# HaokunChen245/FedDAT

Hardware: AMD Instinct MI355X
Metric: VQA samples/sec, ViLT-B/32 dual-adapter local step (higher is better)
Workload: dtype fp16; 1 GPU; configs[1] with fp16 operands (BASELINE.json's configs[1] string says bf16: same operand width and MFMA rate; the bf16 step is in other_operand_format with --full): ViLT-B/32 FedDAT, 1 client per MI355X, fp16 MFMA operands (dynamic loss scale, GradScaler semantics on the device, initial 2^14), fp32 accumulate / masters, batch=32/client, 384x384 synthetic + 40-token questions, MKD on; batch_per_client=32, seq_len=185, clients=1, hip_graph=True, ranks=1, hetero_steps=False

## Files before the change

feddat_amd/csrc/common.hip.h:

```cpp
#pragma once
#include <hip/hip_runtime.h>
#include <stdint.h>

#include "../../include/feddat_hip.h"

typedef __bf16 tbf16;
typedef __bf16 tbf16x8 __attribute__((ext_vector_type(8)));
#ifdef FEDDAT_OPERANDS_F16
typedef _Float16 bf16;
#define FD_OPERAND_FORMAT FEDDAT_OPERANDS_FP16
#define FD_MFMA_16X16X32_ASM "v_mfma_f32_16x16x32_f16"
#else
typedef __bf16 bf16;
#define FD_OPERAND_FORMAT FEDDAT_OPERANDS_BF16
#define FD_MFMA_16X16X32_ASM "v_mfma_f32_16x16x32_bf16"
#endif
typedef bf16 bf16x2 __attribute__((ext_vector_type(2)));
typedef bf16 bf16x4 __attribute__((ext_vector_type(4)));
typedef bf16 bf16x8 __attribute__((ext_vector_type(8)));
typedef short s16x4 __attribute__((ext_vector_type(4)));
typedef float f32x4 __attribute__((ext_vector_type(4)));
typedef float f32x2 __attribute__((ext_vector_type(2)));

#define FD_WAVE 64

#if defined(__HIP_DEVICE_COMPILE__) && !defined(__gfx950__)
#error "libfeddat_hip.so is written for gfx950 (MI355X) only: build with --offload-arch=gfx950"
#endif

#define FD_CHECK_ARG(cond)                 \
    do {                                   \
        if (!(cond)) return FEDDAT_EINVAL; \
    } while (0)

#define FD_LAUNCH_RET()                                        \
    do {                                                       \
        hipError_t e__ = hipGetLastError();                    \
        return e__ == hipSuccess ? FEDDAT_OK : FEDDAT_ELAUNCH; \
    } while (0)

int fd_device_cus(int* n_cu);
int fd_set_max_lds(const void* kernel, int bytes);
#ifdef FEDDAT_ABLATE
#define FD_ABL(x) (x)
#else
#define FD_ABL(x) 0
#endif
constexpr unsigned FD_DEBUG_SELECT_BITS = 1u | 2u | 32u | 64u | 128u | 256u | (1u << 23) | (1u << 27) | (0xfu << 28);
int fd_debug_flags();
int fd_prepare_all_kernels();
int fd_prepare_gemm_kernels();
int fd_prepare_attn_kernels();

#define LDS_PTR(p) ((__attribute__((address_space(3))) void*)(p))
#define GLB_PTR(p) ((const __attribute__((address_space(1))) void*)(p))

__device__ __forceinline__ float wave_sum(float v) {
#pragma unroll
    for (int o = 32; o > 0; o >>= 1) v += __shfl_xor(v, o, 64);
    return v;
}
__device__ __forceinline__ float wave_max(float v) {
#pragma unroll
    for (int o = 32; o > 0; o >>= 1) v = fmaxf(v, __shfl_xor(v, o, 64));
    return v;
}
__device__ __forceinline__ bool fd_nonfinite(float x) { return !(fabsf(x) <= __FLT_MAX__); }

__device__ __forceinline__ uint32_t fd_fmix32(uint32_t x) {
    x ^= x >> 16; x *= 0x85EBCA6Bu; x ^= x >> 13; x *= 0xC2B2AE35u; x ^= x >> 16;
    return x;
}
struct FdDrop {
    uint32_t key0, key1s, thr;
    float scale;
};
__device__ __forceinline__ FdDrop fd_drop_make(float p, uint32_t key0, uint32_t key1, const int* step) {
    FdDrop d;
    d.key0 = key0;
    d.key1s = key1 + (step ? (uint32_t)*step : 0u) * 0x632BE5ABu;
    d.thr = (uint32_t)((double)p * 4294967296.0);
    d.scale = 1.0f / (1.0f - p);
    return d;
}
__device__ __forceinline__ bool fd_drop_keep(const FdDrop& d, uint32_t idx) {
    return fd_fmix32(fd_fmix32(idx * 0x9E3779B1u + d.key0) + d.key1s) >= d.thr;
}

__device__ __forceinline__ void erf_exp_f(float u, float& erf_x, float& exp_mx2) {
    const float x = u * 0.70710678118654752f;
    const float ax = fabsf(x);
    const float t = __frcp_rn(1.0f + 0.3275911f * ax);
    exp_mx2 = __expf(-x * x);
    const float poly = t * (0.254829592f + t * (-0.284496736f + t * (1.421413741f + t * (-1.453152027f + t * 1.061405429f))));
    const float e = 1.0f - poly * exp_mx2;
    erf_x = copysignf(e, x);
}
__device__ __forceinline__ float gelu_f(float u) {
    float er, ex;
    erf_exp_f(u, er, ex);
    return 0.5f * u * (1.0f + er);
}
__device__ __forceinline__ float gelu_grad_f(float u) {
    float er, ex;
    erf_exp_f(u, er, ex);
    return 0.5f * (1.0f + er) + u * 0.39894228040143268f * ex;
}

typedef float f32x2 __attribute__((ext_vector_type(2)));
__device__ __forceinline__ f32x2 odd_poly9_pk(f32x2 t, const float (&c)[9]) {
    const f32x2 t2 = t * t;
    f32x2 p = f32x2{c[8], c[8]};
#pragma unroll
    for (int k = 7; k >= 0; --k) p = p * t2 + f32x2{c[k], c[k]};
    return p * t;
}
__device__ __forceinline__ f32x2 clamp_unit_pk(f32x2 u) {
    f32x2 t = u * f32x2{1.0f / 4.5f, 1.0f / 4.5f};
    t[0] = __builtin_amdgcn_fmed3f(t[0], -1.0f, 1.0f);
    t[1] = __builtin_amdgcn_fmed3f(t[1], -1.0f, 1.0f);
    return t;
}
__device__ __forceinline__ f32x2 gelu_pk(f32x2 u) {
    constexpr float C[9] = {3.589798371e+00f, -1.207231863e+01f, 3.590728051e+01f, -8.046883329e+01f, 1.320808609e+02f,
                            -1.519935397e+02f, 1.145676310e+02f, -5.029529085e+01f, 9.684438904e+00f};
    const f32x2 e = odd_poly9_pk(clamp_unit_pk(u), C);
    const f32x2 h = u * f32x2{0.5f, 0.5f};
    return h * e + h;
}
__device__ __forceinline__ f32x2 gelu_grad_pk(f32x2 u) {
    constexpr float C[9] = {3.586068066e+00f, -2.393606056e+01f, 1.043871964e+02f, -2.983035769e+02f, 5.731157980e+02f,
// ... 106 lines not shown
```

feddat_amd/csrc/gemm_bf16.hip:

```cpp
#include <stdlib.h>

#include <type_traits>

#include "common.hip.h"

namespace {

constexpr int BM = 128, BN = 128, BK = 64;
typedef unsigned int u32x4 __attribute__((ext_vector_type(4)));
constexpr int TILE_BYTES = BM * BK * 2;

struct GemmArgs {
    const bf16* A;
    const bf16* B;
    const float* bias;
    const float* resid;
    const bf16* aux;
    float* out_f32;
    bf16* out_bf16;
    bf16* out2_bf16;
    int M, N, K;
    int lda, ldb, ldr, ldaux, ldo32, ldo16, ldo2;
    int epi;
    int nostore;
// ... 227 lines not shown
#pragma unroll
                    for (int j = 0; j < 2; ++j) fb[j] = read_frag(tb, wn * 32 + j * 16 + frow, ks * 4 + fg);
#pragma unroll
                    for (int i = 0; i < 2; ++i)
#pragma unroll
                        for (int j = 0; j < 2; ++j) acc[i][j] = mfma16x32(fb[j], fa[i], acc[i][j]);
                }
            }
            __syncthreads();
        }
    }
    tile_epilogue_dispatch<2, 2>(g, acc, m0 + wm * 32, n0 + wn * 32, g.M, lane);
}


constexpr int V2_BN = 192;
constexpr int V2_TILE_B = V2_BN * BK * 2;
constexpr int V2_EPI_WAVE = 5120;
constexpr int V2_EPI_LD = 208;
template <int WM> struct V2Cfg {
    static constexpr int BM = 64 * WM;
    static constexpr int TILE_A = BM * BK * 2;
    static constexpr int STAGE = TILE_A + V2_TILE_B;
    static constexpr int EPI_OFF = 2 * STAGE;
    static constexpr int LDS = EPI_OFF + 8 * V2_EPI_WAVE;
    static constexpr int NP = WM + 3;
};


struct GemmArgsV2 {
    GemmArgs g;
    int bm;
    int tiles_m;
    int nx, tm_per, tn_per;
    int dbg;
};

__device__ __forceinline__ void v2_tile_coords(const GemmArgsV2& a, int tile_id, int total, int& m0, int& n0,
                                               int& m_last) {
    const int tiles_n = a.g.N / V2_BN;
    int tm, tn;
    if (a.nx == 1) {
        const int q = total >> 3, r8 = total & 7, xcd = tile_id & 7;
        const int wg = (xcd < r8 ? xcd * (q + 1) : r8 * (q + 1) + (xcd - r8) * q) + (tile_id >> 3);
        tm = wg / tiles_n;
        tn = wg - tm * tiles_n;
    } else {
        const int xcd = tile_id & 7, li = tile_id >> 3;
        const int xm = xcd / a.nx, xn = xcd - xm * a.nx;
        const int lm = li / a.tn_per;
        tm = xm * a.tm_per + lm;
        tn = xn * a.tn_per + (li - lm * a.tn_per);
    }
    m0 = tm * a.bm;
    n0 = tn * V2_BN;
    m_last = min(m0 + a.bm, a.g.M) - 1;
}

template <int WM>
__device__ __forceinline__ void v2_piece_ptrs(const GemmArgs& g, int m0, int m_last, int n0, int wave, int lane,
                                              const bf16* (&pa)[WM], const bf16* (&pb)[3]) {
#pragma unroll
    for (int i = 0; i < WM; ++i) {
        const int r = (wave * WM + i) * 8 + (lane >> 3);
        pa[i] = g.A + (size_t)min(m0 + r, m_last) * g.lda + (lane & 7) * 8;
    }
#pragma unroll
    for (int i = 0; i < 3; ++i) {
        const int r = (wave * 3 + i) * 8 + (lane >> 3);
        pb[i] = g.B + (size_t)min(n0 + r, g.N - 1) * g.ldb + (lane & 7) * 8;
    }
}

constexpr int V2_EPI_LD16 = 208;
constexpr int V2_EPI_LD8 = 112;
#ifdef FD_EPI_NT
#define FD_STREAM_STORE(ptr, val) __builtin_nontemporal_store((val), (ptr))
#define FD_STREAM_LOAD(ptr) __builtin_nontemporal_load(ptr)
#else
#define FD_STREAM_STORE(ptr, val) (*(ptr) = (val))
#define FD_STREAM_LOAD(ptr) (*(ptr))
#endif
__device__ uint4 fd_epi_sink[64];
template <int EPI, int WM, bool SINK = false>
__device__ __forceinline__ void v2_epilogue_bf16(const GemmArgs& g, f32x4 (&acc)[WM][6], char* stg, int mbase, int nbase,
                                                 int m_end, int lane) {
    asm volatile("" : "+v"(lane));
    const int frow = lane & 15, fg = lane >> 4;
    constexpr bool G8OUT_ = EPI == FEDDAT_EPI_GELU_G8 || EPI == FEDDAT_EPI_MUL_G8 || EPI == FEDDAT_EPI_GELU_G8_F8 ||
                            EPI == FEDDAT_EPI_MUL_G8_F8;
    constexpr int COLC_OFF = 16 * V2_EPI_LD16;
    static_assert(COLC_OFF + 2 * 384 <= V2_EPI_WAVE, "column constants fit behind the staged slab");
    f32x4 bias4[G8OUT_ ? 1 : 6];
    if (G8OUT_) {
        if (lane < 24) {
            *reinterpret_cast<f32x4*>(stg + COLC_OFF + lane * 16) =
                g.bias ? *reinterpret_cast<const f32x4*>(g.bias + nbase + lane * 4) : f32x4{0.f, 0.f, 0.f, 0.f};
            if (g.sw) *reinterpret_cast<f32x4*>(stg + COLC_OFF + 384 + lane * 16) = *reinterpret_cast<const f32x4*>(g.sw + nbase + lane * 4);
        }
    } else {
#pragma unroll
        for (int j = 0; j < 6; ++j)
            bias4[j] = g.bias ? *reinterpret_cast<const f32x4*>(g.bias + nbase + j * 16 + fg * 4) : f32x4{0.f, 0.f, 0.f, 0.f};
    }
    int srow[3], sc8[3];
#pragma unroll
    for (int p = 0; p < 3; ++p) {
        const int idx = p * 64 + lane;
        srow[p] = idx / 12;
        sc8[p] = idx - srow[p] * 12;
    }
    constexpr bool G8OUT = EPI == FEDDAT_EPI_GELU_G8 || EPI == FEDDAT_EPI_GELU_G8_F8;
    constexpr bool G8IN = EPI == FEDDAT_EPI_MUL_G8 || EPI == FEDDAT_EPI_MUL_G8_F8;
    constexpr bool F8OUT = EPI == FEDDAT_EPI_GELU_G8_F8 || EPI == FEDDAT_EPI_MUL_G8_F8;
    int r8[2], c8[2];
#pragma unroll
    for (int p = 0; p < 2; ++p) {
        const int idx = p * 64 + lane;
        r8[p] = idx / 6;
        c8[p] = idx - r8[p] * 6;
    }
    char* wr8 = stg + frow * V2_EPI_LD8 + fg * 4;
    u32x4 ux8[G8IN ? WM : 1][2];
    auto aux8_load = [&](int i) {
#pragma unroll
        for (int p = 0; p < 2; ++p) {
            const unsigned mc = (unsigned)min(mbase + i * 16 + r8[p], m_end - 1);
            const unsigned off = mc * (unsigned)g.ldaux + (unsigned)(nbase + c8[p] * 16);
            ux8[i][p] = FD_STREAM_LOAD(reinterpret_cast<const u32x4*>(reinterpret_cast<const char*>(g.aux) + off));
        }
    };
    if (G8IN) {
#pragma unroll
        for (int i = 0; i < WM; ++i) aux8_load(i);
    }
    bf16x8 ux[G8IN ? 1 : WM][3];
    auto aux_load = [&](int i) {
#pragma unroll
        for (int p = 0; p < 3; ++p) {
            const unsigned mc = (unsigned)min(mbase + i * 16 + srow[p], m_end - 1);
            const unsigned off = (mc * (unsigned)g.ldaux + (unsigned)(nbase + sc8[p] * 8)) * 2u;
            ux[i][p] = *reinterpret_cast<const bf16x8*>(reinterpret_cast<const char*>(g.aux) + off);
        }
    };
    constexpr int AUX_AHEAD = WM < 4 ? WM : 4;
    if (EPI == FEDDAT_EPI_MUL_DGELU) {
#pragma unroll
        for (int i = 0; i < AUX_AHEAD; ++i) aux_load(i);
    }
    char* wr = stg + frow * V2_EPI_LD16 + fg * 8;
    auto put = [&](bf16* dst, int ld, int i, const f32x4 (&val)[6]) {
#pragma unroll
        for (int j = 0; j < 6; ++j) *reinterpret_cast<bf16x4*>(wr + j * 32) = cvt4(val[j]);
        bf16x8 v[3];
#pragma unroll
        for (int p = 0; p < 3; ++p) v[p] = *reinterpret_cast<const bf16x8*>(stg + srow[p] * V2_EPI_LD16 + sc8[p] * 16);
#pragma unroll
        for (int p = 0; p < 3; ++p) {
            const int m = mbase + i * 16 + srow[p];
            if (SINK) {
                bf16* o = m < m_end ? dst + (size_t)m * ld + nbase + sc8[p] * 8 : reinterpret_cast<bf16*>(fd_epi_sink) + lane * 8;
                *reinterpret_cast<bf16x8*>(o) = v[p];
            } else if (m < m_end && !FD_ABL(g.nostore & 1)) {
                FD_STREAM_STORE(reinterpret_cast<bf16x8*>(dst + (size_t)m * ld + nbase + sc8[p] * 8), v[p]);
            }
        }
    };
    auto slab8_out = [&](uint8_t* o8, int ld, int i) {
        u32x4 cv[2];
#pragma unroll
        for (int p = 0; p < 2; ++p) cv[p] = *reinterpret_cast<const u32x4*>(stg + r8[p] * V2_EPI_LD8 + c8[p] * 16);
#pragma unroll
        for (int p = 0; p < 2; ++p) {
            const int m = mbase + i * 16 + r8[p];
            if (m < m_end && (p == 0 || lane < 32) && !FD_ABL(g.nostore & 1))
                FD_STREAM_STORE(reinterpret_cast<u32x4*>(o8 + (size_t)m * ld + nbase + c8[p] * 16), cv[p]);
        }
    };
    f32x4 sw4[G8OUT_ ? 1 : 6];
    if (g.sw && !G8OUT_) {
#pragma unroll
        for (int j = 0; j < 6; ++j) sw4[j] = *reinterpret_cast<const f32x4*>(g.sw + nbase + j * 16 + fg * 4);
    }
    auto colc = [&](int which, int j) { return *reinterpret_cast<const f32x4*>(stg + COLC_OFF + which * 384 + j * 64 + fg * 16); };
#pragma unroll
    for (int i = 0; i < WM; ++i) {
        f32x4 val[6];
        if (g.sw) {
            const float sa = g.sa ? g.sa[min(mbase + i * 16 + frow, m_end - 1)] : 1.0f;
#pragma unroll
            for (int j = 0; j < 6; ++j) {
                if (EPI == FEDDAT_EPI_MUL_G8_F8)
                    val[j] = acc[i][j] * (colc(1, j) * f32x4{1.0f / FEDDAT_F8_GRAD_HEADROOM, 1.0f / FEDDAT_F8_GRAD_HEADROOM,
                                                              1.0f / FEDDAT_F8_GRAD_HEADROOM, 1.0f / FEDDAT_F8_GRAD_HEADROOM});
                else
                    val[j] = acc[i][j] * ((G8OUT_ ? colc(1, j) : sw4[j]) * f32x4{sa, sa, sa, sa}) + (G8OUT_ ? colc(0, j) : bias4[j]);
            }
        } else {
#pragma unroll
            for (int j = 0; j < 6; ++j) val[j] = acc[i][j] + (G8OUT_ ? colc(0, j) : bias4[j]);
        }
        if (EPI == FEDDAT_EPI_MUL_DGELU) {
#pragma unroll
            for (int p = 0; p < 3; ++p) *reinterpret_cast<bf16x8*>(stg + srow[p] * V2_EPI_LD16 + sc8[p] * 16) = ux[i][p];
#pragma unroll
            for (int j = 0; j < 6; ++j) {
                const bf16x4 u = *reinterpret_cast<const bf16x4*>(wr + j * 32);
                if (!FD_ABL(g.nostore & 2)) val[j] = val[j] * gelu_grad4_pk(f32x4{(float)u[0], (float)u[1], (float)u[2], (float)u[3]});
                else val[j] = val[j] * f32x4{(float)u[0], (float)u[1], (float)u[2], (float)u[3]};
            }
            if (i + AUX_AHEAD < WM) aux_load(i + AUX_AHEAD);
        }
        if (EPI == FEDDAT_EPI_GELU) {
            if (g.out2_bf16) put(g.out2_bf16, g.ldo2, i, val);
#pragma unroll
            for (int j = 0; j < 6; ++j)
                if (!FD_ABL(g.nostore & 2)) val[j] = gelu4_pk(val[j]);
        }
        if (G8IN) {
#pragma unroll
            for (int p = 0; p < 2; ++p) *reinterpret_cast<u32x4*>(stg + r8[p] * V2_EPI_LD8 + c8[p] * 16) = ux8[i][p];
#pragma unroll
            for (int j = 0; j < 6; ++j) val[j] = val[j] * fd_g8_decode4(*reinterpret_cast<const unsigned*>(wr8 + j * 16));
        }
        if (G8OUT) {
#pragma unroll
            for (int j = 0; j < 6; ++j) {
                f32x4 fj, gj;
                gelu_and_grad4_pk(val[j], fj, gj);
                *reinterpret_cast<unsigned*>(wr8 + j * 16) = fd_g8_encode4(FD_ABL(g.nostore & 2) ? val[j] : gj);
                val[j] = fj;
            }
            slab8_out(reinterpret_cast<uint8_t*>(g.out2_bf16), g.ldo2, i);
        }
        if (F8OUT) {
            constexpr float S = EPI == FEDDAT_EPI_GELU_G8_F8 ? 1.0f / FEDDAT_F8_ACT_SCALE : 1.0f;
#pragma unroll
            for (int j = 0; j < 6; ++j) {
                f32x4 x = val[j] * f32x4{S, S, S, S};
#pragma unroll
                for (int e = 0; e < 4; ++e) x[e] = __builtin_amdgcn_fmed3f(x[e], -448.0f, 448.0f);
                int pk = __builtin_amdgcn_cvt_pk_fp8_f32(x[0], x[1], 0, false);
                pk = __builtin_amdgcn_cvt_pk_fp8_f32(x[2], x[3], pk, true);
                *reinterpret_cast<int*>(wr8 + j * 16) = pk;
            }
            slab8_out(reinterpret_cast<uint8_t*>(g.out_bf16), g.ldo16, i);
        } else {
            put(g.out_bf16, g.ldo16, i, val);
        }
    }
}

template <int EPI, int WM, bool DEQ = false>
__device__ __forceinline__ void v2_epilogue(const GemmArgs& g, f32x4 (&acc)[WM][6], char* stg, int mbase, int nbase,
                                            int m_end, int lane) {
    asm volatile("" : "+v"(lane));
    const int frow = lane & 15, fg = lane >> 4;
    f32x4 bias4[6];
#pragma unroll
    for (int j = 0; j < 6; ++j)
        bias4[j] = g.bias ? *reinterpret_cast<const f32x4*>(g.bias + nbase + j * 16 + fg * 4) : f32x4{0.f, 0.f, 0.f, 0.f};
    f32x4 sw4[DEQ ? 6 : 1];
    if (DEQ) {
#pragma unroll
        for (int j = 0; j < 6; ++j) sw4[j] = *reinterpret_cast<const f32x4*>(g.sw + nbase + j * 16 + fg * 4);
    }
    int srow[3], sc4[3];
// ... 94 lines not shown
#endif
    const GemmArgs& g = a.g;
    const int tid = threadIdx.x;
    const int lane = tid & 63;
    const int wave = __builtin_amdgcn_readfirstlane(tid >> 6);
    const int grp = wave >> 2;
    const int wm = wave >> 1, wn = wave & 1;
    const int total = a.tiles_m * (g.N / V2_BN);
    const int grid = gridDim.x, bid = blockIdx.x;
    const int my_tiles = (total - bid + grid - 1) / grid;
    const int nk = g.K / BK;
    const int total_it = my_tiles * nk;

    f32x4 acc[WM][6];
#pragma unroll
    for (int i = 0; i < WM; ++i)
#pragma unroll
        for (int j = 0; j < 6; ++j) acc[i][j] = f32x4{0.f, 0.f, 0.f, 0.f};

    int m0, n0, m_last;
    v2_tile_coords(a, bid, total, m0, n0, m_last);
    V2State<WM> L;
    v2_piece_ptrs<WM>(g, m0, m_last, n0, wave, lane, L.pa, L.pb);
    auto sc_ptr = [&](int tm0, int tml) {
        const int r = wave * (8 * WM) + min(lane, 8 * WM - 1);
        return g.amx + (size_t)min(tm0 + r, tml) * g.ld_mx;
    };
    L.psc = MXA ? sc_ptr(m0, m_last) : nullptr;
    L.l_tile = 0;
    L.l_kt = 0;
    int issued = 0;
    const int lds_lane = (lane >> 3) * 128 + ((((lane & 7) ^ (lane >> 3)) & 7) << 4);

    u32x4 rs[NP];
    int written = 0;
    auto gload_piece = [&](int p) {
        const int koff = L.l_kt * BK;
        rs[p] = *reinterpret_cast<const u32x4*>((p < WM ? L.pa[p < WM ? p : 0] : L.pb[p < WM ? 0 : p - WM]) + koff);
    };
    auto stream_advance = [&]() {
        if (issued + 1 < total_it) {
            if (++L.l_kt == nk) {
                L.l_kt = 0;
                ++L.l_tile;
                int lm0, ln0, lml;
                v2_tile_coords(a, bid + L.l_tile * grid, total, lm0, ln0, lml);
                v2_piece_ptrs<WM>(g, lm0, lml, ln0, wave, lane, L.pa, L.pb);
                if (MXA) L.psc = sc_ptr(lm0, lml);
            }
        }
        ++issued;
    };
    auto lwrite_piece = [&](int p, int stage) {
        char* sb = smem + stage * Cfg::STAGE + lds_lane +
                   (p < WM ? (wave * WM + p) * 1024 : Cfg::TILE_A + (wave * 3 + p - WM) * 1024);
        *reinterpret_cast<u32x4*>(sb) = rs[p];
    };
    unsigned rsc = 0;
    auto gload_sc = [&]() {
        if (MXA) rsc = *reinterpret_cast<const unsigned*>(L.psc + L.l_kt * 4);
    };
    auto lwrite_sc = [&](int stage) {
        if (MXA && lane < 8 * WM) *reinterpret_cast<unsigned*>(smem + SC_OFF + stage * (256 * WM) + (wave * (8 * WM) + lane) * 4) = rsc;
    };
    auto gload = [&]() {
#pragma unroll
        for (int p = 0; p < NP; ++p) gload_piece(p);
        gload_sc();
        stream_advance();
    };
    auto lwrite = [&](int stage) {
#pragma unroll
        for (int p = 0; p < NP; ++p) lwrite_piece(p, stage);
        lwrite_sc(stage);
        ++written;
    };

    const int frow = lane & 15, fg = lane >> 4;
    const int frag_off[2] = {frow * 128 + (((0 + fg) ^ (frow & 7)) << 4), frow * 128 + (((4 + fg) ^ (frow & 7)) << 4)};
    char* stg = smem + Cfg::EPI_OFF + wave * V2_EPI_WAVE;
    int kt = 0, c_tile = 0, st = 0;
    bool pend = false;
    int pm0 = 0, pn0 = 0, pml = 0;
    auto run_epilogue = [&](int em0, int en0, int eml) {
        const int mb = em0 + wm * (16 * WM), nb = en0 + wn * 96, me = eml + 1;
        if (!FD_ABL(a.dbg & 8)) {
            if (EPI == FEDDAT_EPI_BF16 || EPI == FEDDAT_EPI_GELU || EPI == FEDDAT_EPI_MUL_DGELU || EPI == FEDDAT_EPI_GELU_G8 ||
                EPI == FEDDAT_EPI_MUL_G8 || EPI == FEDDAT_EPI_GELU_G8_F8 || EPI == FEDDAT_EPI_MUL_G8_F8)
                v2_epilogue_bf16<EPI, WM>(g, acc, stg, mb, nb, me, lane);
            else
                v2_epilogue<EPI, WM, FP8>(g, acc, stg, mb, nb, me, lane);
        }
#pragma unroll
        for (int i = 0; i < WM; ++i)
#pragma unroll
            for (int j = 0; j < 6; ++j) acc[i][j] = f32x4{0.f, 0.f, 0.f, 0.f};
    };

    gload();
    lwrite(0);
    gload();
    if (grp == 1) {
        lwrite(1);
        gload();
    }
    asm volatile("s_waitcnt lgkmcnt(0)" ::: "memory");
    __builtin_amdgcn_sched_barrier(0);
    __builtin_amdgcn_s_barrier();
    if (grp == 1) __builtin_amdgcn_s_barrier();
    __builtin_amdgcn_sched_barrier(0);

    for (int it = 0; it < total_it; ++it) {
        bf16x8 fa[2][WM], fb[2][6];
        int asc[MXA ? WM : 1];
        auto read_frags = [&]() {
            if (MXA) {
#pragma unroll
                for (int i = 0; i < WM; ++i)
                    asc[i] = *reinterpret_cast<const uint8_t*>(smem + SC_OFF + st * (256 * WM) + (wm * (16 * WM) + i * 16 + frow) * 4 + fg);
            }
            const int a_base = st * Cfg::STAGE + wm * (16 * WM * 128);
            const int b_base = st * Cfg::STAGE + Cfg::TILE_A + wn * (96 * 128);
#pragma unroll
            for (int ks = 0; ks < 2; ++ks) {
                const char* pb_ = smem + (frag_off[ks] + b_base);
                const char* pa_ = smem + (frag_off[ks] + a_base);
#pragma unroll
                for (int j = 0; j < 6; ++j) fb[ks][j] = *reinterpret_cast<const bf16x8*>(pb_ + j * 2048);
#pragma unroll
                for (int i = 0; i < WM; ++i) fa[ks][i] = *reinterpret_cast<const bf16x8*>(pa_ + i * 2048);
                __builtin_amdgcn_sched_barrier(0);
            }
        };
        const bool boundary = pend;
        if (boundary && grp == 0) {
            __builtin_amdgcn_sched_barrier(0);
            __builtin_amdgcn_s_barrier();
            __builtin_amdgcn_sched_barrier(0);
        }
        if (boundary) {
            run_epilogue(pm0, pn0, pml);
            pend = false;
            if (grp == 1) {
                __builtin_amdgcn_sched_barrier(0);
                __builtin_amdgcn_s_barrier();
                __builtin_amdgcn_sched_barrier(0);
            }
        }
        read_frags();
        asm volatile("s_waitcnt lgkmcnt(0)" ::: "memory");
        __builtin_amdgcn_sched_barrier(0);
        __builtin_amdgcn_s_barrier();
        __builtin_amdgcn_sched_barrier(0);
        const int wstage = written & 1;
        __builtin_amdgcn_s_setprio(1);
        if constexpr (FP8 && !FP8_K32) {
#pragma unroll
            for (int i = 0; i < WM; ++i) {
#pragma unroll
                for (int j = 0; j < 6; ++j)
                    acc[i][j] = MXA ? mfma16x128_fp8_mx_sb(fb[0][j], fb[1][j], fa[0][i], fa[1][i], acc[i][j], asc[MXA ? i : 0])
                                    : mfma16x128_fp8_mx(fb[0][j], fb[1][j], fa[0][i], fa[1][i], acc[i][j]);
                __builtin_amdgcn_sched_barrier(0);
#pragma unroll
                for (int p = 2 * i; p < 2 * i + 2; ++p)
                    if (p < NP) {
                        lwrite_piece(p, wstage);
                        gload_piece(p);
                    }
                if (MXA && i == WM - 1) {
                    lwrite_sc(wstage);
                    gload_sc();
                }
                __builtin_amdgcn_sched_barrier(0);
            }
        } else {
#pragma unroll
        for (int ks = 0; ks < 2; ++ks)
#pragma unroll
            for (int i = 0; i < WM; ++i) {
#pragma unroll
                for (int j = 0; j < 6; ++j)
                    acc[i][j] = FP8 ? mfma16x64_fp8(fb[ks][j], fa[ks][i], acc[i][j]) : mfma16x32(fb[ks][j], fa[ks][i], acc[i][j]);
                __builtin_amdgcn_sched_barrier(0);
                if (ks * WM + i < NP) {
                    lwrite_piece(ks * WM + i, wstage);
                    gload_piece(ks * WM + i);
                }
                __builtin_amdgcn_sched_barrier(0);
            }
        }
        __builtin_amdgcn_s_setprio(0);
        ++written;
        stream_advance();
        asm volatile("s_waitcnt lgkmcnt(0)" ::: "memory");
        st ^= 1;
        if (++kt == nk) {
            kt = 0;
            pend = true; pm0 = m0; pn0 = n0; pml = m_last;
            if (++c_tile < my_tiles) v2_tile_coords(a, bid + c_tile * grid, total, m0, n0, m_last);
        }
        __builtin_amdgcn_sched_barrier(0);
        __builtin_amdgcn_s_barrier();
        __builtin_amdgcn_sched_barrier(0);
    }
    if (grp == 0) __builtin_amdgcn_s_barrier();
    __builtin_amdgcn_sched_barrier(0);
    if (pend) run_epilogue(pm0, pn0, pml);
}





__device__ __forceinline__ void mfma_agpr(f32x4& c, const bf16x8& a, const bf16x8& b) {
    asm volatile(FD_MFMA_16X16X32_ASM " %0, %1, %2, %0" : "+a"(c) : "v"(a), "v"(b));
}
__device__ __forceinline__ void mfma_agpr_first(f32x4& c, const bf16x8& a, const bf16x8& b) {
    asm volatile(FD_MFMA_16X16X32_ASM " %0, %1, %2, 0" : "=a"(c) : "v"(a), "v"(b));
}

__device__ __forceinline__ void mfma_vgpr(f32x4& c, const bf16x8& a, const bf16x8& b) {
    asm volatile(FD_MFMA_16X16X32_ASM " %0, %1, %2, %0" : "+v"(c) : "v"(a), "v"(b));
}
__device__ __forceinline__ void mfma_vgpr_first(f32x4& c, const bf16x8& a, const bf16x8& b) {
    asm volatile(FD_MFMA_16X16X32_ASM " %0, %1, %2, 0" : "=v"(c) : "v"(a), "v"(b));
}

template <int RT> struct V3Cfg {
    static constexpr int BM = 32 * RT;
    static constexpr int TILE_A = BM * BK * 2;
    static constexpr int STAGE = TILE_A + V2_TILE_B;
    static constexpr int EPI_OFF = 2 * STAGE;
    static constexpr int LDS = EPI_OFF + 4 * V2_EPI_WAVE;
    static constexpr int NP = RT + 6;
};

template <int EPI, int RT, int FAKE = 0, bool DUAL = false>
__global__ __launch_bounds__(256, DUAL ? 2 : 1) void gemm_nt_v3_kernel(GemmArgsV2 a) {
    using Cfg = V3Cfg<RT>;
    static_assert(!DUAL || (RT == 4 && 4 * V2_EPI_WAVE <= Cfg::STAGE), "the dual form: 128-row tiles, staging inside one stage");
    constexpr int NP = Cfg::NP, NM = 6 * RT;
    constexpr int LH0 = (NM - 2 * NP) < NP ? (NM - 2 * NP) : NP;
    static_assert(LH0 >= 0 && NP - LH0 <= 12, "writes fit half 0, deferred reloads fit ahead of half 1's fragment reads");
    extern __shared__ __attribute__((aligned(16))) char smem[];
#ifdef FEDDAT_ABLATE
    if (const int q = (a.dbg >> 24) & 7) {
        const long t0 = wall_clock64(), d = (long)((blockIdx.x >> 3) & 3) * q * 200;
        while (wall_clock64() - t0 < d) __builtin_amdgcn_s_sleep(8);
    }
#endif
    const GemmArgs& g = a.g;
    const int tid = threadIdx.x;
    const int lane = tid & 63;
    const int wave = __builtin_amdgcn_readfirstlane(tid >> 6);
    const int wm = wave >> 1, wn = wave & 1;
    const int total = a.tiles_m * (g.N / V2_BN);
    const int grid = gridDim.x, bid = blockIdx.x;
    const int my_tiles = (total - bid + grid - 1) / grid;
    const int nk = g.K / BK;
    const int total_it = my_tiles * nk;

    f32x4 acc[RT][6];
    int m0, n0, m_last;
    v2_tile_coords(a, bid, total, m0, n0, m_last);
    unsigned pp[NP];
    auto piece_ptrs = [&](int tm0, int tml, int tn0) {
#pragma unroll
        for (int i = 0; i < RT; ++i) {
            const int r = (wave * RT + i) * 8 + (lane >> 3);
            pp[i] = ((unsigned)min(tm0 + r, tml) * (unsigned)g.lda + (lane & 7) * 8) * 2u;
        }
#pragma unroll
        for (int i = 0; i < 6; ++i) {
            const int r = (wave * 6 + i) * 8 + (lane >> 3);
            pp[RT + i] = ((unsigned)min(tn0 + r, g.N - 1) * (unsigned)g.ldb + (lane & 7) * 8) * 2u;
        }
    };
    piece_ptrs(m0, m_last, n0);
    int l_tile = 0, l_kt = 0, issued = 0;
    const int lds_lane = (lane >> 3) * 128 + ((((lane & 7) ^ (lane >> 3)) & 7) << 4);
    u32x4 rs[NP];
    auto gload_piece = [&](int p) {
        const char* base = reinterpret_cast<const char*>(p < RT ? g.A : g.B) + (size_t)l_kt * (BK * 2);
        rs[p] = *reinterpret_cast<const u32x4*>(base + pp[p]);
    };
    auto stream_advance = [&]() {
        if (issued + 1 < total_it) {
            if (++l_kt == nk) {
// ... 513 lines not shown
                                  const float* b_scale, int M, int N, int K, int epi, const float* bias, const void* aux,
                                  int ldaux, void* out_bf16, int ldo16, void* out2_bf16, int ldo2, hipStream_t stream) {
    FD_CHECK_ARG(A8 && B8 && a_scale && b_scale && out_bf16 && M >= 1024 && N > 0 && N % V2_BN == 0 && K > 0 && K % 128 == 0);
    const bool g8in = epi == FEDDAT_EPI_MUL_G8 || epi == FEDDAT_EPI_MUL_G8_F8;
    const bool g8out = epi == FEDDAT_EPI_GELU_G8 || epi == FEDDAT_EPI_GELU_G8_F8;
    const bool f8out = epi == FEDDAT_EPI_GELU_G8_F8 || epi == FEDDAT_EPI_MUL_G8_F8;
    FD_CHECK_ARG(epi == FEDDAT_EPI_BF16 || epi == FEDDAT_EPI_GELU || epi == FEDDAT_EPI_MUL_DGELU || g8in || g8out);
    FD_CHECK_ARG(epi != FEDDAT_EPI_MUL_DGELU || (aux && ldaux % 8 == 0 && ((uintptr_t)aux & 15) == 0 &&
                                                (size_t)M * ldaux * 2 < (1ull << 32)));
    FD_CHECK_ARG(!g8in || (aux && ldaux % 16 == 0 && ldaux >= N && ((uintptr_t)aux & 15) == 0 && (size_t)M * ldaux < (1ull << 32)));
    FD_CHECK_ARG(!g8out || (out2_bf16 && ldo2 % 16 == 0 && ldo2 >= N));
    FD_CHECK_ARG(lda % 16 == 0 && ldb % 16 == 0 && lda >= K && ldb >= K && ((uintptr_t)out_bf16 & 15) == 0);
    FD_CHECK_ARG(f8out ? (ldo16 % 16 == 0 && ldo16 >= N) : ldo16 % 8 == 0);
    FD_CHECK_ARG(!out2_bf16 || (ldo2 % 8 == 0 && ((uintptr_t)out2_bf16 & 15) == 0));
    GemmArgs g = fp8_args(A8, lda, a_scale, B8, ldb, b_scale, M, N, K, epi, bias);
    g.aux = (const bf16*)aux; g.ldaux = ldaux;
    g.out_bf16 = (bf16*)out_bf16; g.out2_bf16 = (bf16*)out2_bf16; g.ldo16 = ldo16; g.ldo2 = ldo2;
    return fp8_launch(g, K, stream);
}

extern "C" int feddat_gemm_fp8_nt_f32(const void* A8, int lda, const float* a_scale, const void* B8, int ldb,
                                      const float* b_scale, int M, int N, int K, const float* bias, const float* resid,
                                      int ldr, float* out_f32, int ldo32, hipStream_t stream) {
    FD_CHECK_ARG(A8 && B8 && a_scale && b_scale && out_f32 && M >= 1024 && N > 0 && N % V2_BN == 0 && K > 0 && K % 128 == 0);
    FD_CHECK_ARG(lda % 16 == 0 && ldb % 16 == 0 && lda >= K && ldb >= K && ldo32 % 4 == 0 && ldo32 >= N);
    FD_CHECK_ARG(!resid || (ldr % 4 == 0 && ldr >= N && (size_t)M * ldr * 4 < (1ull << 32)));
    GemmArgs g = fp8_args(A8, lda, a_scale, B8, ldb, b_scale, M, N, K, resid ? FEDDAT_EPI_RESID_F32 : FEDDAT_EPI_F32, bias);
    g.resid = resid; g.ldr = ldr; g.out_f32 = out_f32; g.ldo32 = ldo32;
    return fp8_launch(g, K, stream);
}

extern "C" int feddat_gemm_bf16_nt(const void* A, int lda, const void* B, int ldb, int M, int N, int K, int epi,
                                   const float* bias, const float* resid, int ldr, const void* aux, int ldaux,
                                   float* out_f32, int ldo32, void* out_bf16, int ldo16, void* out2_bf16, int ldo2,
                                   hipStream_t stream) {
    FD_CHECK_ARG(A && B && M > 0 && N > 0 && K > 0);
    FD_CHECK_ARG(lda % 8 == 0 && ldb % 8 == 0 && lda >= K && ldb >= K);
    const int flags = fd_debug_flags();
    int n_cu = 0;
    if (fd_device_cus(&n_cu) != FEDDAT_OK) return FEDDAT_ELAUNCH;
    GemmRoute r;
    FD_CHECK_ARG(fd_gemm_route(M, N, K, epi, FEDDAT_GEMM_OP16, n_cu, flags, r) == FEDDAT_OK);
    const bool use_v2 = r.family >= FEDDAT_GEMM_V2;
    switch (epi) {
        case FEDDAT_EPI_BF16: FD_CHECK_ARG(out_bf16 && ldo16 % 4 == 0); break;
        case FEDDAT_EPI_RESID_F32:
            FD_CHECK_ARG(out_f32 && resid && ldr % 4 == 0 && ldo32 % 4 == 0 && (size_t)M * ldr * 4 < (1ull << 32));
            break;
        case FEDDAT_EPI_GELU: FD_CHECK_ARG(out_bf16 && ldo16 % 4 == 0 && (!out2_bf16 || ldo2 % 4 == 0)); break;
        case FEDDAT_EPI_MUL_DGELU:
            FD_CHECK_ARG(out_bf16 && aux && ldaux % 4 == 0 && ldo16 % 4 == 0 && (size_t)M * ldaux * 2 < (1ull << 32));
            break;
        case FEDDAT_EPI_F32: FD_CHECK_ARG(out_f32 && ldo32 % 4 == 0); break;
        case FEDDAT_EPI_GELU_G8:
            FD_CHECK_ARG(use_v2 && out_bf16 && out2_bf16 && ldo2 % 16 == 0 && ldo2 >= N && ((uintptr_t)out2_bf16 & 15) == 0);
            break;
        case FEDDAT_EPI_MUL_G8:
            FD_CHECK_ARG(use_v2 && out_bf16 && aux && ldaux % 16 == 0 && ldaux >= N && ((uintptr_t)aux & 15) == 0 &&
                         (size_t)M * ldaux < (1ull << 32));
            break;
        default: return FEDDAT_EINVAL;
    }
    if (use_v2) {
        if (epi != FEDDAT_EPI_RESID_F32 && epi != FEDDAT_EPI_F32) FD_CHECK_ARG(ldo16 % 8 == 0 && ((uintptr_t)out_bf16 & 15) == 0);
        if (epi == FEDDAT_EPI_GELU && out2_bf16) FD_CHECK_ARG(ldo2 % 8 == 0 && ((uintptr_t)out2_bf16 & 15) == 0);
        if (epi == FEDDAT_EPI_MUL_DGELU) FD_CHECK_ARG(ldaux % 8 == 0 && ((uintptr_t)aux & 15) == 0);
    }
    GemmArgs g{};
    g.A = (const bf16*)A; g.B = (const bf16*)B; g.bias = bias; g.resid = resid; g.aux = (const bf16*)aux;
    g.out_f32 = out_f32; g.out_bf16 = (bf16*)out_bf16; g.out2_bf16 = (bf16*)out2_bf16;
    g.M = M; g.N = N; g.K = K; g.lda = lda; g.ldb = ldb; g.ldr = ldr; g.ldaux = ldaux;
    g.ldo32 = ldo32; g.ldo16 = ldo16; g.ldo2 = ldo2; g.epi = epi;
    g.nostore = FD_ABL(((flags & 16) ? 1 : 0) | ((flags & 4) ? 2 : 0));
    if (!use_v2) return gemm_launch(r.family == FEDDAT_GEMM_MID ? gemm_nt_mid_kernel : gemm_nt_kernel, r, r.grid, g, stream);
    int variant = GK_PLAIN, grid = r.grid;
#ifdef FEDDAT_ABLATE
    if ((r.dbg & 512) && r.family != FEDDAT_GEMM_DUAL) {
        const int dbg = r.dbg;
        FD_CHECK_ARG(fd_gemm_route(M, N, K, epi, FEDDAT_GEMM_OP16, n_cu, (dbg & ~(1 | 64)) | 2 | 32 | 128, r) == FEDDAT_OK);
        r.dbg = dbg;
        variant = GK_DEFER_PROBE;
        grid = r.grid;
    }
    const int cap = (r.dbg >> 8) & 0xfff;
    if (r.family == FEDDAT_GEMM_V2 && cap > 0 && cap < grid) grid = cap;
#endif
    return gemm_launch_persistent(g, r, FEDDAT_GEMM_OP16, variant, 0, grid, stream);
}
```

Measured before the change: 4514 samples/s.

## Skew GELU_G8/MUL_G8 epilogue to interleave per-row math with stores across wave groups

For the two-group persistent GEMM with GELU_G8 or MUL_G8 epilogues, adds a skewed epilogue. It computes the math for row-block i+1 while row-block i is being written out. The group-0 barrier moves inside the epilogue, placed after the first row-block's math or before it, so one group's epilogue math overlaps the other group's stores or MMA. A debug bit selects the lead variant, which can also raise wave priority during math. This changes barrier placement between the two wave groups, so a mismatch could deadlock or serialise, and the extra live registers for the pipelined values may add pressure.

```diff
diff --git a/feddat_amd/csrc/common.hip.h b/feddat_amd/csrc/common.hip.h
--- a/feddat_amd/csrc/common.hip.h
+++ b/feddat_amd/csrc/common.hip.h
@@ -46,7 +46,8 @@
 #else
 #define FD_ABL(x) 0
 #endif
-constexpr unsigned FD_DEBUG_SELECT_BITS = 1u | 2u | 32u | 64u | 128u | 256u | (1u << 23) | (1u << 27) | (0xfu << 28);
+constexpr unsigned FD_DEBUG_EPI_SKEW = 1u << 19;
+constexpr unsigned FD_DEBUG_SELECT_BITS = 1u | 2u | 32u | 64u | 128u | 256u | FD_DEBUG_EPI_SKEW | (1u << 23) | (1u << 27) | (0xfu << 28);
 int fd_debug_flags();
 int fd_prepare_all_kernels();
 int fd_prepare_gemm_kernels();
diff --git a/feddat_amd/csrc/gemm_bf16.hip b/feddat_amd/csrc/gemm_bf16.hip
--- a/feddat_amd/csrc/gemm_bf16.hip
+++ b/feddat_amd/csrc/gemm_bf16.hip
@@ -333,9 +333,9 @@
 #define FD_STREAM_LOAD(ptr) (*(ptr))
 #endif
 __device__ uint4 fd_epi_sink[64];
-template <int EPI, int WM, bool SINK = false>
+template <int EPI, int WM, bool SINK = false, bool SKEW = false>
 __device__ __forceinline__ void v2_epilogue_bf16(const GemmArgs& g, f32x4 (&acc)[WM][6], char* stg, int mbase, int nbase,
-                                                 int m_end, int lane) {
+                                                 int m_end, int lane, int lead = 0) {
     asm volatile("" : "+v"(lane));
     const int frow = lane & 15, fg = lane >> 4;
     constexpr bool G8OUT_ = EPI == FEDDAT_EPI_GELU_G8 || EPI == FEDDAT_EPI_MUL_G8 || EPI == FEDDAT_EPI_GELU_G8_F8 ||
@@ -434,6 +434,72 @@
         for (int j = 0; j < 6; ++j) sw4[j] = *reinterpret_cast<const f32x4*>(g.sw + nbase + j * 16 + fg * 4);
     }
     auto colc = [&](int which, int j) { return *reinterpret_cast<const f32x4*>(stg + COLC_OFF + which * 384 + j * 64 + fg * 16); };
+    if constexpr (SKEW) {
+        static_assert((G8OUT || G8IN) && !F8OUT && !SINK, "skewed form: GELU_G8 / MUL_G8 of the two-group kernel");
+        bf16x4 h[6];
+        unsigned code[G8OUT ? 6 : 1];
+        auto math = [&](int i) {
+            f32x4 val[6];
+#pragma unroll
+            for (int j = 0; j < 6; ++j) val[j] = acc[i][j] + colc(0, j);
+            if (G8IN) {
+#pragma unroll
+                for (int p = 0; p < 2; ++p) *reinterpret_cast<u32x4*>(stg + r8[p] * V2_EPI_LD8 + c8[p] * 16) = ux8[G8IN ? i : 0][p];
+#pragma unroll
+                for (int j = 0; j < 6; ++j) val[j] = val[j] * fd_g8_decode4(*reinterpret_cast<const unsigned*>(wr8 + j * 16));
+            }
+            if (G8OUT) {
+#pragma unroll
+                for (int j = 0; j < 6; ++j) {
+                    f32x4 fj, gj;
+                    gelu_and_grad4_pk(val[j], fj, gj);
+                    code[j] = fd_g8_encode4(FD_ABL(g.nostore & 2) ? val[j] : gj);
+                    val[j] = fj;
+                }
+            }
+#pragma unroll
+            for (int j = 0; j < 6; ++j) h[j] = cvt4(val[j]);
+        };
+        auto out = [&](int i) {
+            if (G8OUT) {
+#pragma unroll
+                for (int j = 0; j < 6; ++j) *reinterpret_cast<unsigned*>(wr8 + j * 16) = code[G8OUT ? j : 0];
+                slab8_out(reinterpret_cast<uint8_t*>(g.out2_bf16), g.ldo2, i);
+            }
+#pragma unroll
+            for (int j = 0; j < 6; ++j) *reinterpret_cast<bf16x4*>(wr + j * 32) = h[j];
+            bf16x8 v[3];
+#pragma unroll
+            for (int p = 0; p < 3; ++p) v[p] = *reinterpret_cast<const bf16x8*>(stg + srow[p] * V2_EPI_LD16 + sc8[p] * 16);
+#pragma unroll
+            for (int p = 0; p < 3; ++p) {
+                const int m = mbase + i * 16 + srow[p];
+                if (m < m_end && !FD_ABL(g.nostore & 1))
+                    FD_STREAM_STORE(reinterpret_cast<bf16x8*>(g.out_bf16 + (size_t)m * g.ldo16 + nbase + sc8[p] * 8), v[p]);
+            }
+        };
+        auto barrier = [&]() {
+            __builtin_amdgcn_sched_barrier(0);
+            __builtin_amdgcn_s_barrier();
+            __builtin_amdgcn_sched_barrier(0);
+        };
+        const bool hi_math = lead == 2;
+        if (lead == 1) barrier();
+        math(0);
+        if (lead == 2) barrier();
+#pragma unroll
+        for (int i = 0; i < WM; ++i) {
+            out(i);
+            __builtin_amdgcn_sched_barrier(0);
+            if (i + 1 < WM) {
+                if (hi_math) __builtin_amdgcn_s_setprio(1);
+                math(i + 1);
+                if (hi_math) __builtin_amdgcn_s_setprio(0);
+                __builtin_amdgcn_sched_barrier(0);
+            }
+        }
+        return;
+    }
 #pragma unroll
     for (int i = 0; i < WM; ++i) {
         f32x4 val[6];
@@ -694,9 +760,19 @@
     int kt = 0, c_tile = 0, st = 0;
     bool pend = false;
     int pm0 = 0, pn0 = 0, pml = 0;
+    constexpr bool SKEW = !FP8 && (EPI == FEDDAT_EPI_GELU_G8 || EPI == FEDDAT_EPI_MUL_G8);
+    const int lead0 = (a.dbg & FD_DEBUG_EPI_SKEW) ? 2 : 1;
     auto run_epilogue = [&](int em0, int en0, int eml) {
         const int mb = em0 + wm * (16 * WM), nb = en0 + wn * 96, me = eml + 1;
-        if (!FD_ABL(a.dbg & 8)) {
+        if constexpr (SKEW) {
+            if (!FD_ABL(a.dbg & 8)) {
+                v2_epilogue_bf16<EPI, WM, false, true>(g, acc, stg, mb, nb, me, lane, grp == 0 ? lead0 : 0);
+            } else if (grp == 0) {
+                __builtin_amdgcn_sched_barrier(0);
+                __builtin_amdgcn_s_barrier();
+                __builtin_amdgcn_sched_barrier(0);
+            }
+        } else if (!FD_ABL(a.dbg & 8)) {
             if (EPI == FEDDAT_EPI_BF16 || EPI == FEDDAT_EPI_GELU || EPI == FEDDAT_EPI_MUL_DGELU || EPI == FEDDAT_EPI_GELU_G8 ||
                 EPI == FEDDAT_EPI_MUL_G8 || EPI == FEDDAT_EPI_GELU_G8_F8 || EPI == FEDDAT_EPI_MUL_G8_F8)
                 v2_epilogue_bf16<EPI, WM>(g, acc, stg, mb, nb, me, lane);
@@ -745,7 +821,7 @@
             }
         };
         const bool boundary = pend;
-        if (boundary && grp == 0) {
+        if (!SKEW && boundary && grp == 0) {
             __builtin_amdgcn_sched_barrier(0);
             __builtin_amdgcn_s_barrier();
             __builtin_amdgcn_sched_barrier(0);
@@ -816,7 +892,7 @@
         __builtin_amdgcn_s_barrier();
         __builtin_amdgcn_sched_barrier(0);
     }
-    if (grp == 0) __builtin_amdgcn_s_barrier();
+    if ((!SKEW || !pend) && grp == 0) __builtin_amdgcn_s_barrier();
     __builtin_amdgcn_sched_barrier(0);
     if (pend) run_epilogue(pm0, pn0, pml);
 }
@@ -1496,7 +1572,7 @@
         variant = GK_DEFER_PROBE;
         grid = r.grid;
     }
-    const int cap = (r.dbg >> 8) & 0xfff;
+    const int cap = (r.dbg >> 8) & 0x7ff;
     if (r.family == FEDDAT_GEMM_V2 && cap > 0 && cap < grid) grid = cap;
 #endif
     return gemm_launch_persistent(g, r, FEDDAT_GEMM_OP16, variant, 0, grid, stream);
```

Result: no change. 4522 samples/s, median of 5 (+0.2%).
